# facebookresearch/PartDistillation

Measured on AMD Instinct MI355X. Metric: images/sec training step, R50 Mask2Former 1024² bs=2/GPU, 1/2/4/8 MI355X, higher is better.
Workload: dtype bf16

## Files before the change

include/pd_gemm.h:

```cpp
#ifndef PD_GEMM_H
#define PD_GEMM_H

#include <stdint.h>

#ifdef __cplusplus
extern "C" {
#endif

int pd_gemm_tn_f32(const float *A, const float *B, const float *bias, float *C, int M, int N, int K, int lda, int ldb,
                   int ldc, int relu, void *stream);

int pd_gemm_tn_f32x3(const float *A, const float *B, const float *bias, float *C, int M, int N, int K, int lda, int ldb,
                     int ldc, int relu, void *stream);

int pd_gemm_wgrad_f32(const float *dY, const float *X, float *dW, float *dB, int M, int N, int K, int ldy, int ldx,
                      int ldw, void *stream);

int pd_gemm_wgrad_acc_f32(const float *dY, const float *X, float *dW, float *dB, int M, int N, int K, int ldy, int ldx,
                          int ldw, void *stream);

int64_t pd_gemm_tn_f32x3_relu_bits_words(int M, int N);
int pd_split3_bf16(const float *W, int N, int K, int ldw, int transpose, void *planes, void *stream);
int pd_gemm_tn_f32x3_pre(const float *A, const void *Bplanes, const float *bias, float *C, uint32_t *bits, float *colsum, int M, int N, int K,
                         int lda, int ldc, int mode, void *stream);
// ... 22 lines not shown
int pd_conv3x3_wgrad_nhwc_f32x3(const float *dY, const float *X, float *dWk, float *dB, float *workspace, int64_t workspace_floats, int B, int H,
                                int W, int Ci, int Co, void *stream);

int pd_conv3x3_nhwc_f32x3(const float *X, const float *Wk, const float *bias, float *Y, int B, int H, int W, int Ci, int Co,
                          void *stream);

int64_t pd_gemm_wgrad_f16x2_ws_floats(int N, int K);
int pd_gemm_wgrad_f16x2_takes_wide_tiles(int N, int K);
int64_t pd_gemm_wgrad_f16x2_grouped_ws_floats(const PdGemmWgradDesc *descs, int count);
int pd_gemm_wgrad_acc_f16x2_ws(const float *dY, const float *X, float *dW, float *dB, const float *y_amax, const float *x_amax,
                               float *workspace, int64_t workspace_floats, int M, int N, int K, int ldy, int ldx, int ldw, void *stream);
int pd_gemm_wgrad_f16x2_grouped(const PdGemmWgradDesc *descs, int count, void *table_host_pinned, void *table_device, float *workspace,
                                int64_t workspace_floats, void *stream);
int pd_conv3x3_wgrad_nhwc_f16x2(const float *dY, const float *X, float *dWk, float *dB, const float *y_amax, const float *x_amax,
                                float *workspace, int64_t workspace_floats, int B, int H, int W, int Ci, int Co, void *stream);
int pd_gemm_tn_f16x2_which(int M, int N, int K, int mode, int has_bits, int has_amax);

int pd_conv3x3_nhwc_f16x2(const float *X, const float *Wk, const float *bias, float *Y, const float *x_amax, const float *w_amax, float *y_amax,
                          int B, int H, int W, int Ci, int Co, void *stream);
int64_t pd_gemm_tn_f16x2_bits_words(int M, int N);
int pd_gemm_tn_f16x2(const float *A, const float *B, const float *bias, float *C, uint32_t *bits, float *colsum, const float *a_amax,
                     const float *b_amax, float *c_amax, int M, int N, int K, int lda, int ldb, int ldc, int mode, void *stream);
int pd_row_amax_f32(const float *X, int rows, int cols, int ld, float *out, void *stream);
int pd_gemm_tn_f16x2_bf16out(const float *A, const float *B, const float *bias, void *C_bf16, const float *a_amax, const float *b_amax, int M, int N,
                             int K, int lda, int ldb, int ldc, void *stream);
int pd_cast_bf16_f32_amax(const void *X_bf16, int rows, int cols, float *Y, float *row_amax, void *stream);

#ifdef __cplusplus
}
#endif
#endif
```

partdistillation_amd/csrc/cmdbuf.hip:

```cpp
#include <hip/hip_runtime.h>
#include <stdint.h>
#include <string.h>

#include <type_traits>
#include <utility>

#include "pd_common.h"
#include "pd_cmdbuf.h"
#include "pd_attention.h"
#include "pd_conv.h"
#include "pd_declayer.h"
#include "pd_criterion.h"
#include "pd_fused.h"
#include "pd_gemm.h"
#include "pd_grouping.h"
#include "pd_igemm.h"
#include "pd_input.h"
#include "pd_kmeans.h"
#include "pd_msda.h"
#include "pd_mx8.h"
#include "pd_optim.h"
#include "pd_rowwise.h"
#include "pd_smallgemm.h"
#include "pd_stem.h"
// ... 38 lines not shown
  PD_E(pd_affine_act_bwd2_bf16),
  PD_E(pd_affine_act_bwd_bf16),
  PD_E(pd_affine_act_fwd_bf16),
  PD_E(pd_attn_bwd_d32),
  PD_E(pd_attn_fwd_d32),
  PD_E(pd_attn_mask_u8),
  PD_E(pd_cast_bf16_f32_amax),
  PD_E(pd_colsum_acc),
  PD_E(pd_conv3x3_nhwc_f16x2),
  PD_E(pd_conv3x3_nhwc_f32x3),
  PD_E(pd_conv3x3_wgrad_nhwc_f16x2),
  PD_E(pd_conv3x3_wgrad_nhwc_f32x3),
  PD_E(pd_conv_bf16_dgrad),
  PD_E(pd_conv_bf16_fwd),
  PD_E(pd_conv_bf16_wgrad),
  PD_E(pd_conv_bf16_wgrad_grouped),
  PD_E(pd_dec_bwd_a),
  PD_E(pd_dec_bwd_b),
  PD_E(pd_dec_fwd_a),
  PD_E(pd_dec_fwd_b),
  PD_E(pd_dec_pack_grouped),
  PD_E(pd_decoder_head_bf16),
  PD_E(pd_filter_transpose_grouped),
  PD_E(pd_gemm_tn_f16x2),
  PD_E(pd_gemm_tn_f16x2_bf16out),
  PD_E(pd_gemm_tn_f32),
  PD_E(pd_gemm_tn_f32x3),
  PD_E(pd_gemm_tn_f32x3_pre),
  PD_E(pd_gemm_tn_f32x3_relu_bits),
  PD_E(pd_gemm_tn_f32x3_relumask),
  PD_E(pd_gemm_wgrad_acc_f16x2_ws),
  PD_E(pd_gemm_wgrad_acc_f32),
  PD_E(pd_gemm_wgrad_acc_f32x3),
  PD_E(pd_gemm_wgrad_acc_f32x3_ws),
  PD_E(pd_gemm_wgrad_f16x2_grouped),
  PD_E(pd_gemm_wgrad_f32),
  PD_E(pd_gemm_wgrad_f32x3_grouped),
  PD_E(pd_gn_coeffs_bwd),
  PD_E(pd_gn_coeffs_fwd),
  PD_E(pd_igemm_bf16),
  PD_E(pd_igemm_bf16_seq),
  PD_E(pd_kmeans_assign),
  PD_E(pd_kmeans_assign_bounded),
  PD_E(pd_kmeans_assign_partial),
  PD_E(pd_kmeans_reduce),
  PD_E(pd_kmeans_reduce_update),
// ... 133 lines not shown
```

partdistillation_amd/csrc/common.hip:

```cpp
#include <hip/hip_runtime.h>
#include <stdarg.h>
#include <stdio.h>
#include <string.h>

#include "pd_common.h"
#include "pd_msda.h"

namespace {
thread_local char g_err[512] = {0};
}

int pd_set_error(int code, const char *fmt, ...)
{
  va_list ap;
  va_start(ap, fmt);
  vsnprintf(g_err, sizeof(g_err), fmt, ap);
  va_end(ap);
  return code;
}

int pd_check_launch(const char *what)
{
  hipError_t e = hipGetLastError();
  if (e == hipSuccess) return PD_OK;
  return pd_set_error(PD_ERR_LAUNCH, "%s: %s", what, hipGetErrorString(e));
}

extern "C" const char *pd_last_error(void) { return g_err; }
extern "C" int pd_abi_version(void) { return 39; }

extern int g_pd_dbg_atomic_scope;
extern int g_pd_dbg_force_generic;
extern int g_pd_dbg_ablate;
extern int g_pd_dbg_x3_narrow;
extern int g_pd_dbg_f16x2;
extern int g_pd_dbg_wgrad_wide;
extern "C" void pd_dbg_set_wgrad_xcd(int v);
extern "C" void pd_dbg_set_wgrad_fast(int v);
extern int g_pd_dbg_bwd_variant;
extern int g_pd_dbg_msda_gate_pct;
extern int g_pd_dbg_wgrad_wgs;
extern int g_pd_dbg_bwd_threads;
extern int g_pd_dbg_attn_scalar;
extern int g_pd_dbg_wattn;
extern int g_pd_dbg_x3;
extern int g_pd_dbg_kmeans;
extern int g_pd_dbg_conv_group_rows;
extern int g_pd_dbg_conv_xcd_major;
extern int g_pd_dbg_sgemm_deep;
extern int g_ig_bn, g_ig_nst, g_ig_splits, g_ig_patch, g_ig_pcls;
extern int g_mx_bn, g_mx_nst;
extern int g_swin_ln_abl;
// ... 43 lines not shown
```

partdistillation_amd/csrc/gemm_f16x2.hip:

```cpp
#include <hip/hip_runtime.h>
#include <stdint.h>
#include <stdlib.h>
#include <type_traits>

#include "f16x2.h"
#include "pd_common.h"
#include "xcd.h"
#include "pd_gemm.h"
#include "pd_msda.h"

#ifndef PD_ABL
#define PD_ABL 0
#endif

namespace {
using namespace pdh2;
__device__ __forceinline__ int xcd_chunk(int bid, int nb) { return pd_xcd_chunk(bid, nb); }
__device__ __forceinline__ unsigned short f2bf_rne(float f)
{
  unsigned u = __float_as_uint(f);
  if ((u & 0x7fffffffu) > 0x7f800000u) return (unsigned short)((u >> 16) | 0x40u);
  u += 0x7fffu + ((u >> 16) & 1u);
  return (unsigned short)(u >> 16);
}
// ... 333 lines not shown
  for (int c = lane * 8; c < cols; c += 512) {
    const uint4 u = *reinterpret_cast<const uint4 *>(p + c);
    float f[8];
    f[0] = __uint_as_float(u.x << 16); f[1] = __uint_as_float(u.x & 0xffff0000u); f[2] = __uint_as_float(u.y << 16); f[3] = __uint_as_float(u.y & 0xffff0000u);
    f[4] = __uint_as_float(u.z << 16); f[5] = __uint_as_float(u.z & 0xffff0000u); f[6] = __uint_as_float(u.w << 16); f[7] = __uint_as_float(u.w & 0xffff0000u);
#pragma unroll
    for (int k = 0; k < 8; ++k) v = fmaxf(v, fabsf(f[k]));
    *reinterpret_cast<float4 *>(q + c) = make_float4(f[0], f[1], f[2], f[3]);
    *reinterpret_cast<float4 *>(q + c + 4) = make_float4(f[4], f[5], f[6], f[7]);
  }
#pragma unroll
  for (int o = 32; o; o >>= 1) v = fmaxf(v, __shfl_xor(v, o, 64));
  if (lane == 0) out[row] = v;
}

constexpr int RS_PANEL = 528, RS_PLANE = 32 * RS_PANEL, RS_BUF = 2 * RS_PLANE;
typedef unsigned u32x4 __attribute__((ext_vector_type(4)));

#ifdef PD_ROWS_PACKED_SPLIT
#define ROWS_SPLIT split4h
#else
#define ROWS_SPLIT split4h_u
#endif
__device__ int g_rows_wstage = 1;
template <bool AM, int MODE = 0>
__global__ __launch_bounds__(512)
void gemm_rows_f16x2_k256(const float *__restrict__ A, const float *__restrict__ B, const float *__restrict__ bias, float *__restrict__ C,
                          int M, int npanels, int lda, int ldb, int ldc, const float *__restrict__ a_amax,
                          const float *__restrict__ b_amax, unsigned *__restrict__ c_amax, unsigned short *__restrict__ bits = nullptr,
                          float *__restrict__ colsum = nullptr)
{
  __shared__ __attribute__((aligned(16))) unsigned char lds0[RS_BUF], lds1[RS_BUF];
  __shared__ __attribute__((aligned(16))) float sinv0[32], sinv1[32], sdump[64];
  const int t = threadIdx.x, lane = t & 63, w = __builtin_amdgcn_readfirstlane(t >> 6), fr = lane & 31, fh = lane >> 5;
  const int x = blockIdx.x & 7, q = blockIdx.x >> 3;
  const int panel = q % npanels, rg = (q / npanels) * 8 + x, nrg = (gridDim.x / 8 / npanels) * 8;
  const int ntile = (M + 31) >> 5;
  const int t0 = (int)((int64_t)rg * ntile / nrg), t1 = (int)((int64_t)(rg + 1) * ntile / nrg), T = t1 - t0;
  if (T <= 0) return;
  const int n0 = panel * 256 + w * 32;

  float4 R[2][4];
  float am[2][4];
  auto gload = [&](int rs, int tile) {
    tile = min(tile, t1 - 1);
#pragma unroll
    for (int j = 0; j < 4; ++j) {
      const int row = min(tile * 32 + w + 8 * j, M - 1);
      if (PD_ABL & 8) R[rs][j] = make_float4(1.f, 0.5f, 0.25f, (float)row);
      else R[rs][j] = *reinterpret_cast<const float4 *>(A + (int64_t)row * lda + 4 * lane);
      am[rs][j] = AM ? a_amax[row] : 0.f;
    }
  };
  auto split_store = [&](int rs, int buf) {
    float invs[4];
#pragma unroll
// ... 42 lines not shown
          const float2 f0 = *reinterpret_cast<const float2 *>(wsrc + 16 * sq), f1 = *reinterpret_cast<const float2 *>(wsrc + 16 * sq + 2), \
                       f2 = *reinterpret_cast<const float2 *>(wsrc + 16 * sq + 4), f3 = *reinterpret_cast<const float2 *>(wsrc + 16 * sq + 6); \
          const SplitH u = split4h(make_float4(f0.x, f0.y, f1.x, f1.y), sbv), v = split4h(make_float4(f2.x, f2.y, f3.x, f3.y), sbv); \
          bh[4 * R + sq] = __builtin_bit_cast(h16x8, u32x4{u.hi.x, u.hi.y, v.hi.x, v.hi.y});                                   \
          bl[4 * R + sq] = __builtin_bit_cast(h16x8, u32x4{u.lo.x, u.lo.y, v.lo.x, v.lo.y});                                   \
        }                                                                                                                      \
        asm volatile("s_waitcnt lgkmcnt(0)" ::: "memory");        \
      }
      PD_WPASS(0, wa, wb) PD_WPASS(1, wb, wa) PD_WPASS(2, wa, wb) PD_WPASS(3, wb, wa)
#undef PD_WPASS
      __syncthreads();
    } else {
      const float *bp = B + (int64_t)(n0 + fr) * ldb + 8 * fh;
#pragma unroll
      for (int s = 0; s < 16; ++s) {
        const SplitH u = split4h((PD_ABL & 64) ? make_float4(1.f, 2.f, (float)s, sbv) : *reinterpret_cast<const float4 *>(bp + 16 * s), sbv),
                     v = split4h((PD_ABL & 64) ? make_float4(1.f, 2.f, (float)s, ibv) : *reinterpret_cast<const float4 *>(bp + 16 * s + 4), sbv);
        bh[s] = __builtin_bit_cast(h16x8, u32x4{u.hi.x, u.hi.y, v.hi.x, v.hi.y});
        bl[s] = __builtin_bit_cast(h16x8, u32x4{u.lo.x, u.lo.y, v.lo.x, v.lo.y});
      }
    }
  }
  const float bv = bias ? bias[n0 + fr] : 0.f;
  float csum = 0.f;
  split_store(0, 0);
  gload(0, t0 + 2);
  __syncthreads();

  auto iter = [&](int it, int par) {
    const unsigned char *base = (par ? lds1 : lds0) + fh * RS_PANEL + fr * 16;
    unsigned wbits = 0u;
    if (MODE == 2) wbits = (unsigned)bits[(((int64_t)(t0 + it) * npanels + panel) * 8 + w) * 64 + lane];
    f32x16 acc0, acc1;
#pragma unroll
    for (int e = 0; e < 16; ++e) { acc0[e] = 0.f; acc1[e] = 0.f; }
#pragma unroll
    for (int s = 0; s < ((PD_ABL & 1) ? 0 : 16); ++s) {
      const h16x8 ah = (PD_ABL & 2) ? bl[15 - s] : *reinterpret_cast<const h16x8 *>(base + 2 * s * RS_PANEL);
      const h16x8 al = (PD_ABL & 2) ? bh[15 - s] : *reinterpret_cast<const h16x8 *>(base + 2 * s * RS_PANEL + RS_PLANE);
#ifdef PD_ROWS_TWO_CHAINS
      if (s & 1) { mmah(acc1, al, bh[s]); mmah(acc0, ah, bl[s]); mmah(acc1, ah, bh[s]); }
      else       { mmah(acc0, al, bh[s]); mmah(acc1, ah, bl[s]); mmah(acc0, ah, bh[s]); }
#else
      mmah(acc0, al, bh[s]); mmah(acc0, ah, bl[s]); mmah(acc0, ah, bh[s]);
#endif
    }
    split_store(par ^ 1, par ^ 1);
    gload(par ^ 1, t0 + it + 3);
#pragma unroll
    for (int s = 0; s < 16; ++s) {
      __builtin_amdgcn_sched_group_barrier(0x008, 1, 0);
      __builtin_amdgcn_sched_group_barrier(0x002, 2, 0);
      __builtin_amdgcn_sched_group_barrier(0x008, 1, 0);
      __builtin_amdgcn_sched_group_barrier(0x002, 2, 0);
      __builtin_amdgcn_sched_group_barrier(0x008, 1, 0);
      __builtin_amdgcn_sched_group_barrier(0x002, 2, 0);
      if (s & 1) __builtin_amdgcn_sched_group_barrier(0x200, 1, 0);
      if ((s & 3) == 3) __builtin_amdgcn_sched_group_barrier(0x020, 1, 0);
    }
    __builtin_amdgcn_sched_barrier(0);
    const int row0 = (t0 + it) * 32;
    float o[16];
#pragma unroll
    for (int qd = 0; qd < 4; ++qd) {
      const float4 ia = *reinterpret_cast<const float4 *>((par ? sinv1 : sinv0) + 8 * qd + 4 * fh);
      o[4 * qd + 0] = (acc0[4 * qd + 0] + acc1[4 * qd + 0]) * (ia.x * ibv) + bv;
      o[4 * qd + 1] = (acc0[4 * qd + 1] + acc1[4 * qd + 1]) * (ia.y * ibv) + bv;
      o[4 * qd + 2] = (acc0[4 * qd + 2] + acc1[4 * qd + 2]) * (ia.z * ibv) + bv;
      o[4 * qd + 3] = (acc0[4 * qd + 3] + acc1[4 * qd + 3]) * (ia.w * ibv) + bv;
    }
    if (MODE != 0) {
      const int64_t widx = (((int64_t)(t0 + it) * npanels + panel) * 8 + w) * 64 + lane;
      unsigned word = 0u;
      if (MODE == 2) { asm volatile("" : "+v"(wbits)); word = wbits; }
#pragma unroll
      for (int e = 0; e < 16; ++e) {
        const int rl = (e & 3) + 8 * (e >> 2) + 4 * fh;
        if (MODE == 1) {
          o[e] = fmaxf(o[e], 0.f);
          word |= (o[e] > 0.f ? 1u : 0u) << e;
        } else {
          o[e] = ((word >> e) & 1u) ? o[e] : 0.f;
          if (row0 + rl < M) csum += o[e];
        }
      }
      if (MODE == 1 && bits) bits[widx] = (unsigned short)word;
    }
    float *cp = C + (int64_t)row0 * ldc + n0 + fr;
    if (PD_ABL & 16) {
#pragma unroll
      for (int e = 0; e < 16; ++e) asm volatile("" ::"v"(o[e]));
    } else if (row0 + 32 <= M) {
#pragma unroll
      for (int e = 0; e < 16; ++e) cp[(int64_t)((e & 3) + 8 * (e >> 2) + 4 * fh) * ldc] = o[e];
    } else {
#pragma unroll
      for (int e = 0; e < 16; ++e) {
        const int rl = (e & 3) + 8 * (e >> 2) + 4 * fh;
        if (row0 + rl < M) cp[(int64_t)rl * ldc] = o[e];
      }
    }
    if (c_amax) {
      float v[16];
#pragma unroll
      for (int e = 0; e < 16; ++e) v[e] = fabsf(o[e]);
#pragma unroll
      for (int n = 8, m = 16; n >= 1; n >>= 1, m >>= 1) {
        const bool up = (lane & m) != 0;
#pragma unroll
        for (int i = 0; i < n; ++i) {
          const float mine = up ? v[n + i] : v[i], send = up ? v[i] : v[n + i];
          v[i] = fmaxf(mine, __shfl_xor(send, m, 64));
        }
      }
      const float r = fmaxf(v[0], __shfl_xor(v[0], 1, 64));
      const int e = (lane >> 1) & 15, rl = (e & 3) + 8 * (e >> 2) + 4 * fh;
      if (!(lane & 1) && row0 + rl < M && r > 0.f) atomicMax(c_amax + row0 + rl, __float_as_uint(r));
    }
    __syncthreads();
  };
  for (int it = 0; it < T; it += 2) {
    iter(it, 0);
    if (it + 1 < T) iter(it + 1, 1);
  }
  if (MODE == 2) {
    csum += __shfl_xor(csum, 32, 64);
    if (lane < 32 && csum != 0.f) unsafeAtomicAdd(colsum + n0 + fr, csum);
  }
}


constexpr int KR_RB = 192, KR_KC = 32;
constexpr int KR_APANEL = KR_RB * 16 + 16, KR_APLANE = (KR_KC / 8) * KR_APANEL, KR_ABUF = 2 * KR_APLANE;
constexpr int KR_BPANEL = 256 * 16 + 16, KR_BPLANE = (KR_KC / 8) * KR_BPANEL, KR_BBUF = 2 * KR_BPLANE;
#ifdef PD_PROBES
constexpr size_t KR_LDS = (size_t)2 * (KR_ABUF + KR_BBUF) + KR_RB * sizeof(float);
#endif

constexpr size_t KP_LDS = (size_t)2 * (KR_ABUF + KR_BBUF) + 2 * KR_RB * sizeof(float) + 4 * sizeof(int);

#ifdef PD_PROBES
#include "../../tools/probes/gemm_f16x2_optin.h"
#endif
__device__ unsigned long long g_kp_trace[2][64][8];
__device__ __forceinline__ void kp_stamp(int role, int chunk, int ev)
{
  if (chunk < 64) g_kp_trace[role][chunk][ev] = __builtin_readcyclecounter();
// ... 489 lines not shown
#ifdef PD_PROBES
  if ((dbg == 90 || (dbg >= 100 && dbg < 132)) && mode == 0 && K == 256 && M >= 4096 && (N % 32) == 0 && N >= 96 && ((N % 128) == 0 || (N % 96) == 0)) return 3;
#endif
  if (dbg != 62 && dbg != 3 && dbg != 13 && dbg != 70 && (mode == 1 || mode == 2) && has_bits && K == 256 && (N % 256) == 0 && N >= 512 && M >= 8192 && has_amax && g_rows_relu) return 2;
  static const bool kpc_env = []() { const char *e = getenv("PD_H2_KPC"); return !e || e[0] != '0'; }();
  if (((kpc_env && dbg == 0) || dbg == 92 || dbg == 93) && mode == 0 && !has_bits && K >= 512 && (K % KR_KC) == 0 && (N % 256) == 0 && N <= 512 && M >= 8192 && kpc_items_ok(M, N)) return 5;
#ifdef PD_PROBES
  static const bool kres_env = []() { const char *e = getenv("PD_H2_KRES"); return e && e[0] == '1'; }();
  if (((kres_env && dbg == 0) || dbg == 91) && mode == 0 && !has_bits && K >= 512 && (K % KR_KC) == 0 && (N % 256) == 0 && N <= 512 && M >= 8192) return 4;
#endif
  const bool wide_ok = (N % 256) == 0 && M >= 1024;
  const bool by_shape = dbg == 0 || dbg == 61 || dbg == 70 || dbg == 80 || dbg == 62;
  static const bool wide_deepk = []() { const char *e = getenv("PD_H2_WIDE_DEEPK"); return e && e[0] == '1'; }();
  const bool wide = has_bits || dbg == 3 || dbg == 13 || (by_shape && wide_ok && (int64_t)((M + 255) / 256) * (N / 256) >= 128 && (N >= 1024 || (K >= 512 && wide_deepk)));
  return wide ? 1 : 0;
}

extern "C" int pd_gemm_tn_f16x2(const float *A, const float *B, const float *bias, float *C, uint32_t *bits, float *colsum, const float *a_amax,
                                const float *b_amax, float *c_amax, int M, int N, int K, int lda, int ldb, int ldc, int mode, void *stream_)
{
  return gemm_tn_f16x2_impl(A, B, bias, C, bits, colsum, a_amax, b_amax, c_amax, M, N, K, lda, ldb, ldc, mode, stream_, 0);
}

extern "C" int pd_gemm_tn_f16x2_bf16out(const float *A, const float *B, const float *bias, void *C_bf16, const float *a_amax, const float *b_amax,
                                        int M, int N, int K, int lda, int ldb, int ldc, void *stream_)
{
  return gemm_tn_f16x2_impl(A, B, bias, reinterpret_cast<float *>(C_bf16), nullptr, nullptr, a_amax, b_amax, nullptr, M, N, K, lda, ldb, ldc, 0, stream_, 1);
}

extern "C" int pd_cast_bf16_f32_amax(const void *X_bf16, int rows, int cols, float *Y, float *row_amax, void *stream_)
{
  if (rows < 0 || cols <= 0 || (cols & 7)) return pd_set_error(PD_ERR_INVALID_ARG, "pd_cast_bf16_f32_amax: rows=%d cols=%d (a multiple of 8)", rows, cols);
  if (rows == 0) return PD_OK;
  if (!X_bf16 || !Y || !row_amax || ((uintptr_t)X_bf16 & 15) || ((uintptr_t)Y & 15)) return pd_set_error(PD_ERR_INVALID_ARG, "pd_cast_bf16_f32_amax: null / misaligned pointer");
  hipLaunchKernelGGL(cast_bf16_f32_amax, dim3((unsigned)((rows + 3) / 4)), dim3(256), 0, (hipStream_t)stream_, (const unsigned short *)X_bf16, rows, cols, Y,
                     row_amax);
  return pd_check_launch("pd_cast_bf16_f32_amax");
}

extern "C" int pd_conv3x3_nhwc_f16x2(const float *X, const float *Wk, const float *bias, float *Y, const float *x_amax, const float *w_amax,
                                     float *y_amax, int B, int H, int W, int Ci, int Co, void *stream_)
{
  if (B < 0 || H <= 0 || W <= 0 || Ci <= 0 || Co <= 0 || (Ci & 15))
    return pd_set_error(PD_ERR_INVALID_ARG, "pd_conv3x3_nhwc_f16x2: B=%d H=%d W=%d Ci=%d (%% 16) Co=%d", B, H, W, Ci, Co);
  if (B == 0) return PD_OK;
  if (!X || !Wk || !Y || ((uintptr_t)X & 15) || ((uintptr_t)Wk & 15)) return pd_set_error(PD_ERR_INVALID_ARG, "pd_conv3x3_nhwc_f16x2: null / misaligned pointer");
// ... 49 lines not shown
```

partdistillation_amd/functions/encoder_core.py:

```python
import os

import torch
from torch.autograd import Function

from .. import MultiScaleDeformableAttention as MSDA
from .. import lib as _lib
from . import rowwise as rw
from .. import cmdbuf
from . import gemm as _gemm
from .gemm import (WgradQueue, gemm_tn_h2, gemm_tn_x3, gemm_tn_x3_pre, gemm_tn_x3_relu_bits, gemm_tn_x3_relumask, gemm_wgrad_acc,
                   h2_bits_supported, pre_supported, relu_bits_supported, row_amax, split3)

def _timed(kind, fn, *args):
    from ..modeling.pixel_decoder.ops.functions.ms_deform_attn_func import _timed as t
    return t(kind, fn, *args)


def _drop_backward_of(key, rec, cache):
    for k in [k for k in cache if k[0] == "bwd" and k[1] == id(rec)]:
        cache.pop(k)


_RECS = cmdbuf.LRU(int(__import__("os").environ.get("PD_ENCODER_REC_CAP", "6")), _drop_backward_of)


def _msda_timing():
    from ..modeling.pixel_decoder.ops.functions.ms_deform_attn_func import _TIMING as t
    return t


N_LAYER = 16


def msda_prep_fwd(offs, logits, ref, shapes, M, L, P):
# ... 59 lines not shown
    n_oa = oa.shape[1]
    P = n_oa // (3 * M * L)
    both = torch.empty(value.numel() + B * S, dtype=torch.float32, device=value.device)
    gv, d_oa_am = both[:value.numel()].view(value.shape), both[value.numel():]
    d_oa = torch.empty((B * S, n_oa), dtype=torch.float32, device=value.device)
    scratch = torch.empty(B * S * M * L, dtype=torch.float32, device=value.device)
    grad_out = grad_out if grad_out.is_contiguous() else grad_out.contiguous()
    _lib.check(_lib.load().pd_msda_fused_backward(value.data_ptr(), shapes.data_ptr(), lsi.data_ptr(), oa.data_ptr(), oa.stride(0), ref.data_ptr(),
                                                  stats.data_ptr(), out.data_ptr(), grad_out.data_ptr(), gv.data_ptr(), d_oa.data_ptr(), d_oa.stride(0),
                                                  d_oa_am.data_ptr(), scratch.data_ptr(), B, S, M, D, L, S, P, rw._stream()))
    return gv, d_oa, d_oa_am


class EncoderSpec:
    def __init__(self, n_heads, n_levels, n_points, eps, im2col_step, reference_points, spatial_shapes, level_start_index):
        self.M, self.L, self.P, self.eps, self.im2col_step = n_heads, n_levels, n_points, eps, im2col_step
        self.ref, self.shapes, self.lsi = reference_points, spatial_shapes, level_start_index


USE_X3 = True
GROUP_WGRADS = os.environ.get("PD_GROUP_WGRADS", "1") != "0"
X3_PROJ = os.environ.get("PD_X3_PROJ", "1") != "0"
H2_WGRAD = os.environ.get("PD_H2_WGRAD", "1") != "0"
H2 = os.environ.get("PD_H2", "1") != "0"
PRESPLIT = False


def _proj(x, w, b=None):
    if X3_PROJ and USE_X3 and x.is_cuda and x.dtype == torch.float32 and w.dtype == torch.float32 and x.shape[1] % 4 == 0 and x.stride(1) == 1 \
            and x.stride(0) % 4 == 0:
        return gemm_tn_x3(x, w, b)
    return torch.addmm(b, x, w.t()) if b is not None else torch.mm(x, w.t())


def _ffn_gemm(x, w, b=None, relu=False):
    if USE_X3 and x.is_cuda and x.dtype == torch.float32 and w.dtype == torch.float32 and x.shape[1] % 4 == 0:
        return gemm_tn_x3(x, w, b, relu)
    if relu:
        return torch._addmm_activation(b, x, w.t(), use_gelu=False)
    return torch.addmm(b, x, w.t()) if b is not None else torch.mm(x, w.t())


import ctypes as _ct


class _TrProblem(_ct.Structure):
# ... 123 lines not shown
            o += n_off + n_aw
            vp_c, vp_wam = wk[o:o + C], wk_am[o:o + C]
            op_c, op_wam = wk[o + C:o + 2 * C], wk_am[o + C:o + 2 * C]
            l1_c, l1_wam = wk[o + 2 * C:o + 2 * C + n_l1], wk_am[o + 2 * C:o + 2 * C + n_l1]
            value = gemm_tn_h2(x, vp_c, vp_b, a_amax=x_am, b_amax=vp_wam)
            oa = gemm_tn_h2(q, w_oa, b_oa_all[i], a_amax=q_am, b_amax=oa_wam)
            v4 = value.view(B, S, M, C // M)
            fused = fwd_amax and n_off == 2 * n_aw and msda_fused_supported(B, S, M, C // M, L, S, P)
            if fused:
                a_am = a_am_all[i]
                a, stats = _timed("fwd", msda_fused_forward, v4, spec.shapes, spec.lsi, oa, ref, a_am)
                loc6, attn5 = oa, stats
            else:
                loc, attn = msda_prep_fwd(oa[:, :n_off], oa[:, n_off:], ref, spec.shapes, M, L, P)
                loc6, attn5 = loc.view(B, S, M, L, P, 2), attn.view(B, S, M, L, P)
            if fused:
                pass
            elif fwd_amax:
                a_am = a_am_all[i]
                a = _timed("fwd", msda_forward_amax, v4, spec.shapes, spec.lsi, loc6, attn5, spec.im2col_step, a_am).view(T, C)
            else:
                a = _timed("fwd", MSDA.ms_deform_attn_forward, v4, spec.shapes, spec.lsi, loc6, attn5, spec.im2col_step).view(T, C)
                a_am = row_amax(a)
            z1, y1, _, _, m1, r1, y1_am, _ = rw.add_ln_fwd(gemm_tn_h2(a, op_c, op_b, a_amax=a_am, b_amax=op_wam), x, n1_w, n1_b, spec.eps, amax=True)
            h_am = h_am_all[i]
            if h2_bits_supported(T, n_l1):
                h, hbits = gemm_tn_h2(y1, l1_c, l1_b, mode=1, want_bits=True, a_amax=y1_am, b_amax=l1_wam, c_amax=h_am)
            else:
                h, hbits = gemm_tn_h2(y1, l1_c, l1_b, mode=1, a_amax=y1_am, b_amax=l1_wam, c_amax=h_am), None
            ffn2 = gemm_tn_h2(h, l2_all[i * C:(i + 1) * C], l2_b, a_amax=h_am, b_amax=l2_am[i * C:(i + 1) * C])
            last = i == nl - 1
            z2, y2, _, ypos, m2, r2, y2_am, ypos_am = rw.add_ln_fwd(ffn2, y1, n2_w, n2_b, spec.eps, c_dtype=torch.float32,
                                                                     pos=pos2, pos_div=1, want_ypos=not last, amax=True)
            saved.append((x, q, v4, loc6, attn5, a, z1, m1, r1, y1, h, z2, m2, r2, ref if fused else None, hbits))
            saved_am.append((x_am, q_am, a_am, y1_am, h_am))
            x, q, x_am, q_am = y2, ypos, y2_am, ypos_am
        return x, saved, saved_am

    @staticmethod
    def _stack_t(params, nl, j):
        ws = [params[i * N_LAYER + j] for i in range(nl)]
        d = (ws[1].data_ptr() - ws[0].data_ptr()) if nl > 1 else 0
        es = ws[0].element_size()
        if nl > 1 and d != 0 and d % es == 0 and all(w.is_contiguous() and w.shape == ws[0].shape for w in ws) \
                and all(ws[i].data_ptr() - ws[0].data_ptr() == i * d for i in range(nl)) \
                and all(w.untyped_storage().data_ptr() == ws[0].untyped_storage().data_ptr() for w in ws):
            N_, K_ = ws[0].shape
# ... 322 lines not shown
```

partdistillation_amd/functions/gemm.py:

```python
import ctypes

import torch
from torch.autograd import Function

from .. import lib as _lib


def _stream():
    return _lib.current_stream()


def gemm_tn(a, b, bias=None, relu=False):
    if not a.is_cuda:
        raise RuntimeError("pd_gemm_tn_f32 runs on the GPU only (no CPU fallback in partdistillation_amd)")
    assert a.dtype == torch.float32 and b.dtype == torch.float32 and a.stride(1) == 1 and b.stride(1) == 1
    M, K = a.shape
    N = b.shape[0]
    c = torch.empty((M, N), dtype=torch.float32, device=a.device)
    with torch.cuda.device(a.device):
        rc = _lib.load().pd_gemm_tn_f32(a.data_ptr(), b.data_ptr(), bias.data_ptr() if bias is not None else None,
                                        c.data_ptr(), M, N, K, a.stride(0), b.stride(0), N, int(relu), _stream())
    _lib.check(rc)
    return c

# ... 70 lines not shown
    N = b.shape[0]
    assert b.shape[1] == K
    for v, n in ((a_amax, M), (b_amax, N), (c_amax, M)):
        assert v is None or (v.dtype == torch.float32 and v.is_contiguous() and v.numel() == n)
    L = _lib.load()
    c = torch.empty((M, N), dtype=torch.float32, device=a.device)
    if mode == 1 and want_bits:
        bits = torch.empty(int(L.pd_gemm_tn_f16x2_bits_words(M, N)), dtype=torch.int32, device=a.device)
    p = lambda t: t.data_ptr() if t is not None else None
    args = (a.data_ptr(), b.data_ptr(), p(bias), c.data_ptr(), p(bits), p(colsum), p(a_amax), p(b_amax), p(c_amax), M, N, K, a.stride(0), b.stride(0), N, mode,
            _stream())
    if not _TIMING["on"]:
        _lib.check(L.pd_gemm_tn_f16x2(*args))
        return (c, bits) if (mode == 1 and want_bits) else c
    which = int(L.pd_gemm_tn_f16x2_which(M, N, K, mode, int(bits is not None), int(a_amax is not None and b_amax is not None)))
    if which in (4, 5) and c_amax is not None:
        which = 0
    label = (f"gemm_rows_f16x2_k256<true, {mode}>" if which == 2 else f"gemm_ra_f16x2_k256<{mode}>" if which == 3
             else "gemm_kres_f16x2<true, 0>" if which == 4 else "gemm_kpc_f16x2<true, 0, false, false>" if which == 5
             else f"gemm_tn_f16x2<{'256, 256, 128, 16' if which == 1 else '128, 128, 64, 16'}, {mode}>")
    with _timed_fwd(2.0 * M * N * K, label, 4.0 * (M * K + N * K + M * N)):
        _lib.check(L.pd_gemm_tn_f16x2(*args))
    return (c, bits) if (mode == 1 and want_bits) else c


def split3(w, transpose=False):
    assert w.is_cuda and w.dtype == torch.float32 and w.dim() == 2 and w.stride(1) == 1
    N, K = w.shape
    out = torch.empty((3, K, N) if transpose else (3, N, K), dtype=torch.bfloat16, device=w.device)
    _lib.check(_lib.load().pd_split3_bf16(w.data_ptr(), N, K, w.stride(0), int(transpose), out.data_ptr(), _stream()))
    return out


def pre_supported(M, N, K):
    return N % 256 == 0 and K % 16 == 0 and M >= 1024 and (-(-M // 256)) * (N // 256) >= 128


def gemm_tn_x3_pre(a, planes, bias=None, mode=0, bits=None, colsum=None, want_bits=False):
    assert a.is_cuda and a.dtype == torch.float32 and a.stride(1) == 1 and planes.dtype == torch.bfloat16 and planes.is_contiguous()
    M, K = a.shape
    N = planes.shape[1]
    assert planes.shape[2] == K
    L = _lib.load()
    c = torch.empty((M, N), dtype=torch.float32, device=a.device)
    if mode == 1 and want_bits:
        bits = torch.empty(int(L.pd_gemm_tn_f32x3_relu_bits_words(M, N)), dtype=torch.int32, device=a.device)
# ... 237 lines not shown
```

partdistillation_amd/lib.py:

```python
import ctypes
import os
import subprocess

_HERE = os.path.dirname(os.path.abspath(__file__))
LIB_PATH = os.environ.get("PD_LIB_PATH") or os.path.join(_HERE, "libpd_hip.so")
CSRC = os.path.join(_HERE, "csrc")

PD_F32, PD_F64, PD_BF16 = 0, 1, 2
ABI_VERSION = 39

_c_int, _c_vp = ctypes.c_int, ctypes.c_void_p

SIGNATURES = {
    "pd_msda_forward": (_c_int, [_c_vp] * 6 + [_c_int] * 9 + [_c_vp]),
    "pd_msda_backward": (_c_int, [_c_vp] * 9 + [_c_int] * 9 + [_c_vp]),
    "pd_msda_backward_last_gate": (_c_int, [_c_vp]),
    "pd_stem7x7_fwd": (_c_int, [_c_vp, _c_int] + [_c_vp] * 4 + [_c_int] * 4 + [_c_vp]),
    "pd_stem_wgrad_workspace_floats": (ctypes.c_int64, []),
    "pd_stem7x7_wgrad": (_c_int, [_c_vp, _c_int] + [_c_vp] * 4 + [_c_int, _c_vp] + [_c_int] * 4 + [_c_vp]),
    "pd_msda_fused_supported": (_c_int, [_c_int] * 7),
    "pd_msda_fused_forward": (_c_int, [_c_vp] * 4 + [_c_int] + [_c_vp] * 4 + [_c_int] * 7 + [_c_vp]),
    "pd_msda_fused_backward": (_c_int, [_c_vp] * 4 + [_c_int] + [_c_vp] * 6 + [_c_int, _c_vp, _c_vp] + [_c_int] * 7 + [_c_vp]),
    "pd_lsa_batched": (_c_int, [_c_vp] * 4 + [_c_int] * 3 + [_c_vp]),
    "pd_sumsq_accumulate": (_c_int, [_c_vp, ctypes.c_int64, _c_int, _c_vp, _c_vp]),
    "pd_adamw_clipped": (_c_int, [_c_vp] * 4 + [ctypes.c_int64, _c_int] + [ctypes.c_double] * 5 + [_c_int, _c_vp, ctypes.c_double, _c_vp, _c_vp]),
    "pd_gemm_tn_f32": (_c_int, [_c_vp] * 4 + [_c_int] * 7 + [_c_vp]),
    "pd_gemm_tn_f32x3": (_c_int, [_c_vp] * 4 + [_c_int] * 7 + [_c_vp]),
    "pd_gemm_wgrad_f16x2_takes_wide_tiles": (_c_int, [_c_int] * 2),
    "pd_gemm_wgrad_f16x2_ws_floats": (ctypes.c_int64, [_c_int] * 2),
    "pd_gemm_wgrad_f16x2_grouped_ws_floats": (ctypes.c_int64, [_c_vp, _c_int]),
    "pd_gemm_wgrad_acc_f16x2_ws": (_c_int, [_c_vp] * 7 + [ctypes.c_int64] + [_c_int] * 6 + [_c_vp]),
    "pd_gemm_wgrad_f16x2_grouped": (_c_int, [_c_vp, _c_int, _c_vp, _c_vp, _c_vp, ctypes.c_int64, _c_vp]),
    "pd_conv3x3_wgrad_nhwc_f16x2": (_c_int, [_c_vp] * 7 + [ctypes.c_int64] + [_c_int] * 5 + [_c_vp]),
    "pd_conv3x3_nhwc_f16x2": (_c_int, [_c_vp] * 7 + [_c_int] * 5 + [_c_vp]),
    "pd_gemm_tn_f16x2_which": (_c_int, [_c_int] * 6),
    "pd_gemm_tn_f16x2_bits_words": (ctypes.c_int64, [_c_int] * 2),
    "pd_gemm_tn_f16x2": (_c_int, [_c_vp] * 9 + [_c_int] * 7 + [_c_vp]),
    "pd_gemm_tn_f16x2_bf16out": (_c_int, [_c_vp] * 6 + [_c_int] * 6 + [_c_vp]),
    "pd_cast_bf16_f32_amax": (_c_int, [_c_vp, _c_int, _c_int, _c_vp, _c_vp, _c_vp]),
    "pd_row_amax_f32": (_c_int, [_c_vp, _c_int, _c_int, _c_int, _c_vp, _c_vp]),
    "pd_gemm_tn_f32x3_relumask": (_c_int, [_c_vp] * 5 + [_c_int] * 6 + [_c_vp]),
    "pd_gemm_tn_f32x3_relu_bits": (_c_int, [_c_vp] * 5 + [_c_int] * 6 + [_c_vp]),
    "pd_gemm_tn_f32x3_relu_bits_words": (ctypes.c_int64, [_c_int] * 2),
    "pd_split3_bf16": (_c_int, [_c_vp, _c_int, _c_int, _c_int, _c_int, _c_vp, _c_vp]),
    "pd_gemm_tn_f32x3_pre": (_c_int, [_c_vp] * 6 + [_c_int] * 6 + [_c_vp]),
    "pd_gemm_wgrad_f32": (_c_int, [_c_vp] * 4 + [_c_int] * 6 + [_c_vp]),
    "pd_gemm_wgrad_acc_f32": (_c_int, [_c_vp] * 4 + [_c_int] * 6 + [_c_vp]),
    "pd_conv3x3_nhwc_f32x3": (_c_int, [_c_vp] * 4 + [_c_int] * 5 + [_c_vp]),
    "pd_gemm_wgrad_acc_f32x3": (_c_int, [_c_vp] * 4 + [_c_int] * 6 + [_c_vp]),
    "pd_conv3x3_wgrad_nhwc_f32x3": (_c_int, [_c_vp] * 5 + [ctypes.c_int64] + [_c_int] * 5 + [_c_vp]),
    "pd_gemm_wgrad_f32x3_ws_floats": (ctypes.c_int64, [_c_int] * 2),
    "pd_gemm_wgrad_f32x3_grouped_table_bytes": (ctypes.c_int64, [_c_int]),
    "pd_gemm_wgrad_f32x3_grouped_ws_floats": (ctypes.c_int64, [_c_vp, _c_int]),
    "pd_gemm_wgrad_f32x3_grouped": (_c_int, [_c_vp, _c_int, _c_vp, _c_vp, _c_vp, ctypes.c_int64, _c_vp]),
    "pd_gemm_wgrad_acc_f32x3_ws": (_c_int, [_c_vp] * 5 + [ctypes.c_int64] + [_c_int] * 6 + [_c_vp]),
    "pd_adamw_clipped_shadow": (_c_int, [_c_vp] * 5 + [ctypes.c_int64] + [ctypes.c_double] * 5 + [_c_int, _c_vp, ctypes.c_double, _c_vp, _c_vp]),
    "pd_conv_bf16_supported": (_c_int, [_c_int] * 5),
    "pd_conv_bf16_fwd": (_c_int, [_c_vp] * 6 + [_c_int] * 11 + [_c_vp]),
    "pd_conv_bf16_wgrad_workspace_floats": (ctypes.c_int64, [_c_int] * 6),
    "pd_conv_bf16_wgrad": (_c_int, [_c_vp] * 4 + [ctypes.c_int64] + [_c_int] * 10 + [_c_vp]),
# ... 208 lines not shown
```

Before: 109.1.

## Fuse output-projection GEMM with residual add and LayerNorm in encoder layers

Adds a MODE 3 epilogue to the row-panel f16x2 GEMM kernel. It adds the residual, computes per-row mean and rstd through a cross-wave LDS reduction, applies gamma and beta, and writes z, y, the statistics and the row amax in one kernel. The encoder's MSDA output projection uses it when M>=8192 and N=K=256, replacing a GEMM followed by a separate add+LayerNorm kernel and saving one round trip through memory for the intermediate. The cost is extra __syncthreads and register pressure in the GEMM epilogue, plus a strided residual load.

```diff
diff --git a/include/pd_gemm.h b/include/pd_gemm.h
--- a/include/pd_gemm.h
+++ b/include/pd_gemm.h
@@ -68,6 +68,9 @@
 int pd_gemm_tn_f16x2(const float *A, const float *B, const float *bias, float *C, uint32_t *bits, float *colsum, const float *a_amax,
                      const float *b_amax, float *c_amax, int M, int N, int K, int lda, int ldb, int ldc, int mode, void *stream);
 int pd_row_amax_f32(const float *X, int rows, int cols, int ld, float *out, void *stream);
+int pd_gemm_rows_ln_fwd_f16x2(const float *A, const float *B, const float *bias, const float *res, const float *gamma, const float *beta, float eps,
+                              float *z, float *y, float *mean, float *rstd, float *y_amax, const float *a_amax, const float *b_amax, int M, int N,
+                              int K, int lda, int ldb, void *stream);
 int pd_gemm_tn_f16x2_bf16out(const float *A, const float *B, const float *bias, void *C_bf16, const float *a_amax, const float *b_amax, int M, int N,
                              int K, int lda, int ldb, int ldc, void *stream);
 int pd_cast_bf16_f32_amax(const void *X_bf16, int rows, int cols, float *Y, float *row_amax, void *stream);
diff --git a/partdistillation_amd/csrc/cmdbuf.hip b/partdistillation_amd/csrc/cmdbuf.hip
--- a/partdistillation_amd/csrc/cmdbuf.hip
+++ b/partdistillation_amd/csrc/cmdbuf.hip
@@ -84,6 +84,7 @@
   PD_E(pd_dec_pack_grouped),
   PD_E(pd_decoder_head_bf16),
   PD_E(pd_filter_transpose_grouped),
+  PD_E(pd_gemm_rows_ln_fwd_f16x2),
   PD_E(pd_gemm_tn_f16x2),
   PD_E(pd_gemm_tn_f16x2_bf16out),
   PD_E(pd_gemm_tn_f32),
diff --git a/partdistillation_amd/csrc/common.hip b/partdistillation_amd/csrc/common.hip
--- a/partdistillation_amd/csrc/common.hip
+++ b/partdistillation_amd/csrc/common.hip
@@ -27,7 +27,7 @@
 }
 
 extern "C" const char *pd_last_error(void) { return g_err; }
-extern "C" int pd_abi_version(void) { return 39; }
+extern "C" int pd_abi_version(void) { return 40; }
 
 extern int g_pd_dbg_atomic_scope;
 extern int g_pd_dbg_force_generic;
diff --git a/partdistillation_amd/csrc/gemm_f16x2.hip b/partdistillation_amd/csrc/gemm_f16x2.hip
--- a/partdistillation_amd/csrc/gemm_f16x2.hip
+++ b/partdistillation_amd/csrc/gemm_f16x2.hip
@@ -379,16 +379,37 @@
 #else
 #define ROWS_SPLIT split4h_u
 #endif
+struct RowsLn {
+  const float *res, *gamma, *beta;
+  float eps;
+  float *y, *mean, *rstd, *y_amax;
+};
+template <bool MAX>
+__device__ __forceinline__ float half_reduce16(float (&v)[16], int lane)
+{
+#pragma unroll
+  for (int n = 8, m = 16; n >= 1; n >>= 1, m >>= 1) {
+    const bool up = (lane & m) != 0;
+#pragma unroll
+    for (int i = 0; i < n; ++i) {
+      const float mine = up ? v[n + i] : v[i], send = up ? v[i] : v[n + i], got = __shfl_xor(send, m, 64);
+      v[i] = MAX ? fmaxf(mine, got) : mine + got;
+    }
+  }
+  const float got = __shfl_xor(v[0], 1, 64);
+  return MAX ? fmaxf(v[0], got) : v[0] + got;
+}
 __device__ int g_rows_wstage = 1;
 template <bool AM, int MODE = 0>
 __global__ __launch_bounds__(512)
 void gemm_rows_f16x2_k256(const float *__restrict__ A, const float *__restrict__ B, const float *__restrict__ bias, float *__restrict__ C,
                           int M, int npanels, int lda, int ldb, int ldc, const float *__restrict__ a_amax,
                           const float *__restrict__ b_amax, unsigned *__restrict__ c_amax, unsigned short *__restrict__ bits = nullptr,
-                          float *__restrict__ colsum = nullptr)
+                          float *__restrict__ colsum = nullptr, RowsLn ln = RowsLn{})
 {
   __shared__ __attribute__((aligned(16))) unsigned char lds0[RS_BUF], lds1[RS_BUF];
   __shared__ __attribute__((aligned(16))) float sinv0[32], sinv1[32], sdump[64];
+  __shared__ __attribute__((aligned(16))) float lnp1[MODE == 3 ? 256 : 1], lnp2[MODE == 3 ? 256 : 1], lnpm[MODE == 3 ? 256 : 1], lnw[MODE == 3 ? 512 : 1];
   const int t = threadIdx.x, lane = t & 63, w = __builtin_amdgcn_readfirstlane(t >> 6), fr = lane & 31, fh = lane >> 5;
   const int x = blockIdx.x & 7, q = blockIdx.x >> 3;
   const int panel = q % npanels, rg = (q / npanels) * 8 + x, nrg = (gridDim.x / 8 / npanels) * 8;
@@ -477,6 +498,16 @@
     }
   }
   const float bv = bias ? bias[n0 + fr] : 0.f;
+  float lgm = 1.f, lbt = 0.f;
+  if (MODE == 3) { lgm = ln.gamma[n0 + fr]; lbt = ln.beta[n0 + fr]; }
+  auto flush_amax = [&](int tile) {
+    if (w == 0 && lane < 32) {
+      float v = 0.f;
+#pragma unroll
+      for (int k = 0; k < 8; ++k) v = fmaxf(v, lnpm[k * 32 + lane]);
+      if (tile * 32 + lane < M) ln.y_amax[tile * 32 + lane] = v;
+    }
+  };
   float csum = 0.f;
   split_store(0, 0);
   gload(0, t0 + 2);
@@ -486,6 +517,13 @@
     const unsigned char *base = (par ? lds1 : lds0) + fh * RS_PANEL + fr * 16;
     unsigned wbits = 0u;
     if (MODE == 2) wbits = (unsigned)bits[(((int64_t)(t0 + it) * npanels + panel) * 8 + w) * 64 + lane];
+    float rres[16];
+    if (MODE == 3) {
+      if (it > 0) flush_amax(t0 + it - 1);
+      const float *rp = ln.res + n0 + fr;
+#pragma unroll
+      for (int e = 0; e < 16; ++e) rres[e] = rp[(int64_t)min((t0 + it) * 32 + (e & 3) + 8 * (e >> 2) + 4 * fh, M - 1) * 256];
+    }
     f32x16 acc0, acc1;
 #pragma unroll
     for (int e = 0; e < 16; ++e) { acc0[e] = 0.f; acc1[e] = 0.f; }
@@ -524,7 +562,7 @@
       o[4 * qd + 2] = (acc0[4 * qd + 2] + acc1[4 * qd + 2]) * (ia.z * ibv) + bv;
       o[4 * qd + 3] = (acc0[4 * qd + 3] + acc1[4 * qd + 3]) * (ia.w * ibv) + bv;
     }
-    if (MODE != 0) {
+    if (MODE == 1 || MODE == 2) {
       const int64_t widx = (((int64_t)(t0 + it) * npanels + panel) * 8 + w) * 64 + lane;
       unsigned word = 0u;
       if (MODE == 2) { asm volatile("" : "+v"(wbits)); word = wbits; }
@@ -541,19 +579,63 @@
       }
       if (MODE == 1 && bits) bits[widx] = (unsigned short)word;
     }
-    float *cp = C + (int64_t)row0 * ldc + n0 + fr;
-    if (PD_ABL & 16) {
-#pragma unroll
-      for (int e = 0; e < 16; ++e) asm volatile("" ::"v"(o[e]));
-    } else if (row0 + 32 <= M) {
-#pragma unroll
-      for (int e = 0; e < 16; ++e) cp[(int64_t)((e & 3) + 8 * (e >> 2) + 4 * fh) * ldc] = o[e];
-    } else {
-#pragma unroll
-      for (int e = 0; e < 16; ++e) {
-        const int rl = (e & 3) + 8 * (e >> 2) + 4 * fh;
-        if (row0 + rl < M) cp[(int64_t)rl * ldc] = o[e];
-      }
+    if (MODE == 3) {
+#pragma unroll
+      for (int e = 0; e < 16; ++e) o[e] += rres[e];
+    }
+    auto store16 = [&](float *cp, int ld, const float (&val)[16]) {
+      if (PD_ABL & 16) {
+#pragma unroll
+        for (int e = 0; e < 16; ++e) asm volatile("" ::"v"(val[e]));
+      } else if (row0 + 32 <= M) {
+#pragma unroll
+        for (int e = 0; e < 16; ++e) cp[(int64_t)((e & 3) + 8 * (e >> 2) + 4 * fh) * ld] = val[e];
+      } else {
+#pragma unroll
+        for (int e = 0; e < 16; ++e) {
+          const int rl = (e & 3) + 8 * (e >> 2) + 4 * fh;
+          if (row0 + rl < M) cp[(int64_t)rl * ld] = val[e];
+        }
+      }
+    };
+    store16(C + (int64_t)row0 * ldc + n0 + fr, ldc, o);
+    if (MODE == 3) {
+      const int er = (lane >> 1) & 15, rlr = (er & 3) + 8 * (er >> 2) + 4 * fh;
+      auto gather = [&](const float *part) {
+        const float *p = part + fr;
+        return ((p[0] + p[32]) + (p[64] + p[96])) + ((p[128] + p[160]) + (p[192] + p[224]));
+      };
+      auto spread = [&](float *mine, float val, float (&out)[16]) {
+        mine[fr] = val;
+        __builtin_amdgcn_wave_barrier();
+#pragma unroll
+        for (int qd = 0; qd < 4; ++qd) {
+          const float4 m4 = *reinterpret_cast<const float4 *>(mine + 8 * qd + 4 * fh);
+          out[4 * qd + 0] = m4.x; out[4 * qd + 1] = m4.y; out[4 * qd + 2] = m4.z; out[4 * qd + 3] = m4.w;
+        }
+      };
+      float v[16], st[16];
+#pragma unroll
+      for (int e = 0; e < 16; ++e) v[e] = o[e];
+      const float ps = half_reduce16<false>(v, lane);
+      if (!(lane & 1)) lnp1[w * 32 + rlr] = ps;
+      __syncthreads();
+      const float mu = gather(lnp1) * (1.f / 256);
+      if (w == 0 && lane < 32 && row0 + lane < M) ln.mean[row0 + lane] = mu;
+      spread(lnw + w * 64, mu, st);
+#pragma unroll
+      for (int e = 0; e < 16; ++e) { o[e] -= st[e]; v[e] = o[e] * o[e]; }
+      const float pq = half_reduce16<false>(v, lane);
+      if (!(lane & 1)) lnp2[w * 32 + rlr] = pq;
+      __syncthreads();
+      const float rs = rsqrtf(gather(lnp2) * (1.f / 256) + ln.eps);
+      if (w == 0 && lane < 32 && row0 + lane < M) ln.rstd[row0 + lane] = rs;
+      spread(lnw + w * 64 + 32, rs, st);
+#pragma unroll
+      for (int e = 0; e < 16; ++e) { o[e] = o[e] * st[e] * lgm + lbt; v[e] = fabsf(o[e]); }
+      store16(ln.y + (int64_t)row0 * 256 + n0 + fr, 256, o);
+      const float pm = half_reduce16<true>(v, lane);
+      if (!(lane & 1)) lnpm[w * 32 + rlr] = pm;
     }
     if (c_amax) {
       float v[16];
@@ -578,6 +660,7 @@
     iter(it, 0);
     if (it + 1 < T) iter(it + 1, 1);
   }
+  if (MODE == 3) flush_amax(t1 - 1);
   if (MODE == 2) {
     csum += __shfl_xor(csum, 32, 64);
     if (lane < 32 && csum != 0.f) unsafeAtomicAdd(colsum + n0 + fr, csum);
@@ -1113,6 +1196,25 @@
   return gemm_tn_f16x2_impl(A, B, bias, C, bits, colsum, a_amax, b_amax, c_amax, M, N, K, lda, ldb, ldc, mode, stream_, 0);
 }
 
+extern "C" int pd_gemm_rows_ln_fwd_f16x2(const float *A, const float *B, const float *bias, const float *res, const float *gamma, const float *beta,
+                                         float eps, float *z, float *y, float *mean, float *rstd, float *y_amax, const float *a_amax,
+                                         const float *b_amax, int M, int N, int K, int lda, int ldb, void *stream_)
+{
+  if (M < 8192 || N != 256 || K != 256) return pd_set_error(PD_ERR_INVALID_ARG, "pd_gemm_rows_ln_fwd_f16x2: M=%d (>= 8192) N=%d K=%d (256 <- 256 only)", M, N, K);
+  if (!A || !B || !res || !gamma || !beta || !z || !y || !mean || !rstd || !y_amax || !a_amax || !b_amax)
+    return pd_set_error(PD_ERR_INVALID_ARG, "pd_gemm_rows_ln_fwd_f16x2: null pointer");
+  if ((lda & 3) || (ldb & 3) || ((uintptr_t)A & 15) || ((uintptr_t)B & 15))
+    return pd_set_error(PD_ERR_INVALID_ARG, "pd_gemm_rows_ln_fwd_f16x2: lda, ldb must be multiples of 4 and A, B 16-byte aligned");
+  static int ncu = 0;
+  if (!ncu) { int dev = 0; (void)hipGetDevice(&dev); if (hipDeviceGetAttribute(&ncu, hipDeviceAttributeMultiprocessorCount, dev) != hipSuccess || ncu < 8) ncu = 256; }
+  const int G = (ncu / 8) * 8;
+  RowsLn ln;
+  ln.res = res; ln.gamma = gamma; ln.beta = beta; ln.eps = eps; ln.y = y; ln.mean = mean; ln.rstd = rstd; ln.y_amax = y_amax;
+  hipLaunchKernelGGL((gemm_rows_f16x2_k256<true, 3>), dim3((unsigned)G), dim3(512), 0, (hipStream_t)stream_, A, B, bias, z, M, 1, lda, ldb, 256, a_amax,
+                     b_amax, (unsigned *)nullptr, (unsigned short *)nullptr, (float *)nullptr, ln);
+  return pd_check_launch("pd_gemm_rows_ln_fwd_f16x2");
+}
+
 extern "C" int pd_gemm_tn_f16x2_bf16out(const float *A, const float *B, const float *bias, void *C_bf16, const float *a_amax, const float *b_amax,
                                         int M, int N, int K, int lda, int ldb, int ldc, void *stream_)
 {
diff --git a/partdistillation_amd/functions/encoder_core.py b/partdistillation_amd/functions/encoder_core.py
--- a/partdistillation_amd/functions/encoder_core.py
+++ b/partdistillation_amd/functions/encoder_core.py
@@ -8,8 +8,15 @@
 from . import rowwise as rw
 from .. import cmdbuf
 from . import gemm as _gemm
-from .gemm import (WgradQueue, gemm_tn_h2, gemm_tn_x3, gemm_tn_x3_pre, gemm_tn_x3_relu_bits, gemm_tn_x3_relumask, gemm_wgrad_acc,
+from .gemm import (WgradQueue, gemm_rows_ln_fwd, gemm_rows_ln_fwd_supported, gemm_tn_h2, gemm_tn_x3, gemm_tn_x3_pre, gemm_tn_x3_relu_bits, gemm_tn_x3_relumask, gemm_wgrad_acc,
                    h2_bits_supported, pre_supported, relu_bits_supported, row_amax, split3)
+
+def proj_add_ln(a, w, b, res, gamma, beta, eps, a_amax, w_amax):
+    if LN_FUSED and gemm_rows_ln_fwd_supported(a.shape[0], w.shape[0], a.shape[1]):
+        return gemm_rows_ln_fwd(a, w, b, res, gamma, beta, eps, a_amax, w_amax)
+    z, y, _, _, m, r, y_am, _ = rw.add_ln_fwd(gemm_tn_h2(a, w, b, a_amax=a_amax, b_amax=w_amax), res, gamma, beta, eps, amax=True)
+    return z, y, m, r, y_am
+
 
 def _timed(kind, fn, *args):
     from ..modeling.pixel_decoder.ops.functions.ms_deform_attn_func import _timed as t
@@ -115,6 +122,7 @@
 GROUP_WGRADS = os.environ.get("PD_GROUP_WGRADS", "1") != "0"
 X3_PROJ = os.environ.get("PD_X3_PROJ", "1") != "0"
 H2_WGRAD = os.environ.get("PD_H2_WGRAD", "1") != "0"
+LN_FUSED = os.environ.get("PD_ENC_LN_FUSED", "1") != "0"
 H2 = os.environ.get("PD_H2", "1") != "0"
 PRESPLIT = False
 
@@ -284,7 +292,7 @@
             else:
                 a = _timed("fwd", MSDA.ms_deform_attn_forward, v4, spec.shapes, spec.lsi, loc6, attn5, spec.im2col_step).view(T, C)
                 a_am = row_amax(a)
-            z1, y1, _, _, m1, r1, y1_am, _ = rw.add_ln_fwd(gemm_tn_h2(a, op_c, op_b, a_amax=a_am, b_amax=op_wam), x, n1_w, n1_b, spec.eps, amax=True)
+            z1, y1, m1, r1, y1_am = proj_add_ln(a, op_c, op_b, x, n1_w, n1_b, spec.eps, a_am, op_wam)
             h_am = h_am_all[i]
             if h2_bits_supported(T, n_l1):
                 h, hbits = gemm_tn_h2(y1, l1_c, l1_b, mode=1, want_bits=True, a_amax=y1_am, b_amax=l1_wam, c_amax=h_am)
diff --git a/partdistillation_amd/functions/gemm.py b/partdistillation_amd/functions/gemm.py
--- a/partdistillation_amd/functions/gemm.py
+++ b/partdistillation_amd/functions/gemm.py
@@ -116,6 +116,31 @@
     with _timed_fwd(2.0 * M * N * K, label, 4.0 * (M * K + N * K + M * N)):
         _lib.check(L.pd_gemm_tn_f16x2(*args))
     return (c, bits) if (mode == 1 and want_bits) else c
+
+
+def gemm_rows_ln_fwd_supported(M, N, K):
+    return M >= 8192 and N == 256 and K == 256
+
+
+def gemm_rows_ln_fwd(a, b, bias, res, gamma, beta, eps, a_amax, b_amax):
+    if not a.is_cuda:
+        raise RuntimeError("pd_gemm_rows_ln_fwd_f16x2 runs on the GPU only (no CPU fallback in partdistillation_amd)")
+    M, K = a.shape
+    N = b.shape[0]
+    assert a.dtype == torch.float32 and b.dtype == torch.float32 and a.stride(1) == 1 and b.stride(1) == 1 and b.shape[1] == K
+    assert res.dtype == torch.float32 and res.is_contiguous() and res.shape == (M, N)
+    assert gamma.dtype == torch.float32 and beta.dtype == torch.float32 and gamma.numel() == N and beta.numel() == N
+    for v, n in ((a_amax, M), (b_amax, N)):
+        assert v is not None and v.dtype == torch.float32 and v.is_contiguous() and v.numel() == n
+    z = torch.empty((M, N), dtype=torch.float32, device=a.device)
+    y = torch.empty((M, N), dtype=torch.float32, device=a.device)
+    stats = torch.empty((3, M), dtype=torch.float32, device=a.device)
+    args = (a.data_ptr(), b.data_ptr(), bias.data_ptr() if bias is not None else None, res.data_ptr(), gamma.data_ptr(), beta.data_ptr(), float(eps),
+            z.data_ptr(), y.data_ptr(), stats[0].data_ptr(), stats[1].data_ptr(), stats[2].data_ptr(), a_amax.data_ptr(), b_amax.data_ptr(),
+            M, N, K, a.stride(0), b.stride(0), _stream())
+    with _timed_fwd(2.0 * M * N * K, "gemm_rows_f16x2_k256<true, 3>", 4.0 * (M * K + N * K + 3 * M * N)):
+        _lib.check(_lib.load().pd_gemm_rows_ln_fwd_f16x2(*args))
+    return z, y, stats[0], stats[1], stats[2]
 
 
 def split3(w, transpose=False):
diff --git a/partdistillation_amd/lib.py b/partdistillation_amd/lib.py
--- a/partdistillation_amd/lib.py
+++ b/partdistillation_amd/lib.py
@@ -7,7 +7,7 @@
 CSRC = os.path.join(_HERE, "csrc")
 
 PD_F32, PD_F64, PD_BF16 = 0, 1, 2
-ABI_VERSION = 39
+ABI_VERSION = 40
 
 _c_int, _c_vp = ctypes.c_int, ctypes.c_void_p
 
@@ -36,6 +36,7 @@
     "pd_gemm_tn_f16x2_which": (_c_int, [_c_int] * 6),
     "pd_gemm_tn_f16x2_bits_words": (ctypes.c_int64, [_c_int] * 2),
     "pd_gemm_tn_f16x2": (_c_int, [_c_vp] * 9 + [_c_int] * 7 + [_c_vp]),
+    "pd_gemm_rows_ln_fwd_f16x2": (_c_int, [_c_vp] * 6 + [ctypes.c_float] + [_c_vp] * 7 + [_c_int] * 5 + [_c_vp]),
     "pd_gemm_tn_f16x2_bf16out": (_c_int, [_c_vp] * 6 + [_c_int] * 6 + [_c_vp]),
     "pd_cast_bf16_f32_amax": (_c_int, [_c_vp, _c_int, _c_int, _c_vp, _c_vp, _c_vp]),
     "pd_row_amax_f32": (_c_int, [_c_vp, _c_int, _c_int, _c_int, _c_vp, _c_vp]),
```

After: 107.2. 0.983x the previous value.
